# limanling/clip-event

Hardware: AMD Instinct MI355X
Metric: image-text pairs/sec/GPU, ViT-B/32 224px x 77-tok, global-batch contrastive (higher is better)
Workload: dtype bf16; 1 GPU; ViT-B/32 224px x 77-tok, bf16 operands, per-GPU batch 256, K=1, InfoNCE only, full train step (fwd+bwd+clip_grad_norm+Adam), random-init weights; global_batch=256, parallelism=dp1, captions=SOT + U[8,75] random ids + EOT, zero-padded to 77 (SURVEY 8(d) c2), text_rows=live tokens SOT..EOT only: 54.8% of B*77 rows (identical results, see DESIGN.md), fresh_captions_every_step=True, alignment=False, cu_hog=0, nt_pgrid=256, full=False

## Files before the change

clip_event_amd/csrc/gemm.hip:

```cpp
#include <stdlib.h>

#include <map>
#include <mutex>
#include <type_traits>

#include "common.hpp"
#include "nt_plan.hpp"
#include "tn_plan.hpp"
#include "../../include/clip_event_hip.h"

#ifndef CE_DIAG_TN3
#define CE_DIAG_TN3 0
#endif

namespace {

constexpr int NT_BM = 128, NT_BN = 128, NT_BK = 64;
constexpr int NT_STAGE_BYTES = (NT_BM + NT_BN) * NT_BK * 2;
constexpr int NT_LDS_BYTES = 2 * NT_STAGE_BYTES;

#include "gemm_common.hpp"

template <int EPI>
__global__ __launch_bounds__(256, 2) void gemm_nt_kernel(NTArgs p) {
// ... 970 lines not shown
            for (int it = 0; it < 2; ++it) {
                const int es = i * 2 + it;
                f32x4 v0 = *reinterpret_cast<const f32x4*>(ebuf + (it * 8 + e_r) * EROW + e_c * 4);
                f32x4 v1 = *reinterpret_cast<const f32x4*>(ebuf + (it * 8 + e_r) * EROW + e_c * 4 + 16);
                u32x4 a = {0u, 0u, 0u, 0u};
                if constexpr (PF_AUX) {
                    a = ap[es];
                }
                if constexpr (F8) {
                    const float sa = p.sa[min(m0 + e_row + es * 8, p.M - 1)];
                    v0 = v0 * sa * sb0;
                    v1 = v1 * sa * sb1;
                }
                v0 += bias0;
                v1 += bias1;
                if constexpr (EPI == CE_EPI_GELUGRAD_BF16) {
                    f32x4 r0 = {v0[0] * bf_lo(a[0]), v0[1] * bf_hi(a[0]), v0[2] * bf_lo(a[1]), v0[3] * bf_hi(a[1])};
                    f32x4 r1 = {v1[0] * bf_lo(a[2]), v1[1] * bf_hi(a[2]), v1[2] * bf_lo(a[3]), v1[3] * bf_hi(a[3])};
                    cs0 += r0;
                    cs1 += r1;
                    u32x4 o = {pack_bf2(r0[0], r0[1]), pack_bf2(r0[2], r0[3]), pack_bf2(r1[0], r1[1]), pack_bf2(r1[2], r1[3])};
                    epi_bstore16(eo, es, o);
                } else if constexpr (EPI == CE_EPI_BIAS_RESID_F16) {
                    v0 += f16x4_to_f32(u32x2{a[0], a[1]});
                    v1 += f16x4_to_f32(u32x2{a[2], a[3]});
                    const u32x2 h0 = f32_to_f16x4_sat(v0), h1 = f32_to_f16x4_sat(v1);
                    epi_bstore16(eo, es, u32x4{h0[0], h0[1], h1[0], h1[1]});
                } else {
                    nt_epilogue8b<EPI>(eo, eo2, er, es, v0, v1);
                }
            }
        }
        if constexpr (EPI == CE_EPI_GELUGRAD_BF16) {
            if (p.out2) {
                float* colsum = reinterpret_cast<float*>(p.out2);
#pragma unroll
                for (int e = 0; e < 4; ++e) {
#pragma unroll
                    for (int o = 8; o < 64; o <<= 1) {
                        cs0[e] += __shfl_xor(cs0[e], o, 64);
                        cs1[e] += __shfl_xor(cs1[e], o, 64);
                    }
                }
                const int e = lane >> 3;
                const float v = e == 0 ? cs0[0] : e == 1 ? cs0[1] : e == 2 ? cs0[2] : e == 3 ? cs0[3]
                              : e == 4 ? cs1[0] : e == 5 ? cs1[1] : e == 6 ? cs1[2] : cs1[3];
                if (gn + e < p.N) atomicAdd(colsum + gn + e, v);
            }
        }
    };
    for (; cur < list_end; ++t) {
        int tm, tn;
        persist_coords(p, cur, tm, tn);
        if constexpr (TS > 0) {
            if (tm < p.tall_panels) tile_body(std::integral_constant<int, TM>{}, tm, tn);
            else tile_body(std::integral_constant<int, TS>{}, tm, tn);
        } else {
            tile_body(std::integral_constant<int, TM>{}, tm, tn);
        }
        cur = dyn ? __builtin_amdgcn_readfirstlane(tq[(t + 1) & 1]) : cur + walk.step;
    }
}

constexpr int N3_BM = 160, N3_BN = 256, N3_BK = 32, N3_TM = 5;
constexpr int N3_A_BYTES = N3_BM * N3_BK * 2;
constexpr int N3_STAGE_BYTES = (N3_BM + N3_BN) * N3_BK * 2;
constexpr int N3_LDS_BYTES = 2 * N3_STAGE_BYTES;

template <int EPI>
__global__ __launch_bounds__(512, 4) void gemm_nt32_kernel(NTArgs p) {
    extern __shared__ __attribute__((aligned(16))) char smem[];
    const int tid = threadIdx.x;
    const int lane = tid & 63;
    const int wave = __builtin_amdgcn_readfirstlane(tid >> 6);
    const int wm = wave >> 2, wn = wave & 3;

    const int tile = xcd_remap(blockIdx.x, p.tiles_m * p.tiles_n);
    const int tm = tile / p.tiles_n, tn = tile - tm * p.tiles_n;
    const int m0 = tm * N3_BM, n0 = tn * N3_BN;
    const int rowsA = min(p.M - m0, N3_BM), rowsB = min(p.N - n0, N3_BN);
    const u32x4 rA = make_rsrc_words(p.A + (long)m0 * p.lda, (uint32_t)((long)rowsA * p.lda * 2));
    const u32x4 rB = make_rsrc_words(p.B + (long)n0 * p.ldb, (uint32_t)((long)rowsB * p.ldb * 2));

    const int s_row = lane >> 2;
    const int s_chunk = (lane & 3) ^ (((lane >> 5) & 1) << 1);
    const uint32_t vA0 = (uint32_t)((wave * 16 + s_row) * p.lda * 2 + s_chunk * 16);
    const uint32_t vA1 = (uint32_t)(((wave + 8) * 16 + s_row) * p.lda * 2 + s_chunk * 16);
    const uint32_t vB0 = (uint32_t)((wave * 16 + s_row) * p.ldb * 2 + s_chunk * 16);
    const uint32_t vB1 = (uint32_t)(((wave + 8) * 16 + s_row) * p.ldb * 2 + s_chunk * 16);
    const uint32_t lds0 = (uint32_t)(size_t)(lptr_t*)smem;
    auto stage = [&](int st, int kt) {
        const uint32_t base = lds0 + st * N3_STAGE_BYTES;
        const uint32_t kb = (uint32_t)(kt * N3_BK * 2);
        dma16_bounds(rA, base + wave * 1024, vA0 + kb);
        if (wave < 2) dma16_bounds(rA, base + (wave + 8) * 1024, vA1 + kb);
        dma16_bounds(rB, base + N3_A_BYTES + wave * 1024, vB0 + kb);
        dma16_bounds(rB, base + N3_A_BYTES + (wave + 8) * 1024, vB1 + kb);
    };

    f32x4 acc[N3_TM][4];
#pragma unroll
    for (int i = 0; i < N3_TM; ++i)
#pragma unroll
        for (int j = 0; j < 4; ++j) acc[i][j] = f32x4{0.f, 0.f, 0.f, 0.f};

    const int f_pos = (lane >> 4) ^ (((lane >> 3) & 1) << 1);
    const int fa_base = (wm * (N3_TM * 16) + (lane & 15)) * 64 + f_pos * 16;
    const int fb_base = N3_A_BYTES + (wn * 64 + (lane & 15)) * 64 + f_pos * 16;

    const int nk = p.K / N3_BK;
    stage(0, 0);
    asm volatile("s_waitcnt vmcnt(0)" ::: "memory");
    __syncthreads();
    for (int kt = 0; kt < nk; ++kt) {
        const int cur = kt & 1;
        if (kt + 1 < nk) stage(cur ^ 1, kt + 1);
        const char* st = smem + cur * N3_STAGE_BYTES;
        bf16x8 wf[4], af[N3_TM];
#pragma unroll
        for (int t = 0; t < 4; ++t) wf[t] = *reinterpret_cast<const bf16x8*>(st + fb_base + t * 1024);
#pragma unroll
        for (int t = 0; t < N3_TM; ++t) af[t] = *reinterpret_cast<const bf16x8*>(st + fa_base + t * 1024);
#pragma unroll
        for (int t = 0; t < N3_TM; ++t)
#pragma unroll
            for (int nt = 0; nt < 4; ++nt)
                acc[t][nt] = __builtin_amdgcn_mfma_f32_16x16x32_bf16(wf[nt], af[t], acc[t][nt], 0, 0, 0);
        asm volatile("s_waitcnt vmcnt(0)" ::: "memory");
        __syncthreads();
    }

    constexpr int EROW = 272;
    char* ebuf = smem + wave * (16 * EROW);
    const int e_r = lane >> 3, e_c = (lane & 7) * 8;
    const int gn = n0 + wn * 64 + e_c;
    f32x4 bias0 = {0.f, 0.f, 0.f, 0.f}, bias1 = {0.f, 0.f, 0.f, 0.f};
    f32x4 cs0 = {0.f, 0.f, 0.f, 0.f}, cs1 = {0.f, 0.f, 0.f, 0.f};
    if constexpr (epi_has_bias(EPI)) {
        if (gn < p.N) {
            bias0 = *reinterpret_cast<const f32x4*>(p.bias + gn);
            bias1 = *reinterpret_cast<const f32x4*>(p.bias + gn + 4);
        }
    }
#pragma unroll
    for (int t = 0; t < N3_TM; ++t) {
#pragma unroll
        for (int nt = 0; nt < 4; ++nt)
            *reinterpret_cast<f32x4*>(ebuf + (lane & 15) * EROW + (nt * 16 + 4 * (lane >> 4)) * 4) = acc[t][nt];
#pragma unroll
        for (int it = 0; it < 2; ++it) {
            const int m = m0 + wm * (N3_TM * 16) + t * 16 + it * 8 + e_r;
            f32x4 v0 = *reinterpret_cast<const f32x4*>(ebuf + (it * 8 + e_r) * EROW + e_c * 4);
            f32x4 v1 = *reinterpret_cast<const f32x4*>(ebuf + (it * 8 + e_r) * EROW + e_c * 4 + 16);
            if (m < p.M && gn < p.N) {
                v0 += bias0;
                v1 += bias1;
                nt_epilogue8<EPI>(p, m, gn, v0, v1, cs0, cs1);
            }
        }
    }
    if constexpr (EPI == CE_EPI_GELUGRAD_BF16) {
        if (p.out2) wg_colsum_flush(smem, reinterpret_cast<float*>(p.out2), n0, p.N, gn - n0, wm * 8 + e_r, cs0, cs1);
    }
}

constexpr int TN_BN = 128, TN_BK = 128, TN_BM = 64;
constexpr int TN_ROW = 320;
constexpr int TN_TILE_BYTES = TN_BM * TN_ROW;
constexpr int TN_STAGE_BYTES = 2 * TN_TILE_BYTES;
constexpr int TN_LDS_BYTES = 2 * TN_STAGE_BYTES;

struct TNArgs {
    const bf16_t* P; long ldp;
    const bf16_t* Q; long ldq;
    float* out; long ldo;
    int M, Nn, Kk;
    int tiles_n, tiles_k, splits, m_per_split;
};

__device__ __forceinline__ bf16x8 tr_frag(const char* tile, int byte_off) {
    typedef __attribute__((address_space(3))) s16x4 lds_s16x4;
    s16x4 lo = __builtin_amdgcn_ds_read_tr16_b64_v4i16((lds_s16x4*)(tile + byte_off));
    s16x4 hi = __builtin_amdgcn_ds_read_tr16_b64_v4i16((lds_s16x4*)(tile + byte_off + 4 * TN_ROW));
    typedef __attribute__((ext_vector_type(8))) short s16x8;
    s16x8 v = {lo[0], lo[1], lo[2], lo[3], hi[0], hi[1], hi[2], hi[3]};
    return __builtin_bit_cast(bf16x8, v);
}

__global__ __launch_bounds__(256, 2) void gemm_tn_kernel(TNArgs p) {
    extern __shared__ __attribute__((aligned(16))) char smem[];
    const int tid = threadIdx.x;
    const int lane = tid & 63;
    const int wave = __builtin_amdgcn_readfirstlane(tid >> 6);
    const int wn = wave >> 1, wk = wave & 1;

    int bid = blockIdx.x;
    const int split = bid % p.splits;
    bid /= p.splits;
    const int tk = bid % p.tiles_k, tn = bid / p.tiles_k;
    const int n0 = tn * TN_BN, k0 = tk * TN_BK;
    const int ms = split * p.m_per_split;
    const int me = min(p.M, ms + p.m_per_split);
    if (ms >= me) return;
    const int rows = me - ms;

    __amdgpu_buffer_rsrc_t rP = make_rsrc(p.P + (long)ms * p.ldp, (uint32_t)((long)rows * p.ldp * 2));
    __amdgpu_buffer_rsrc_t rQ = make_rsrc(p.Q + (long)ms * p.ldq, (uint32_t)((long)rows * p.ldq * 2));

    const int s_c = tid & 15, s_row = tid >> 4;
    const bool pvalid = (n0 + s_c * 8) < p.Nn, qvalid = (k0 + s_c * 8) < p.Kk;
    const uint32_t gP0 = (uint32_t)(s_row * p.ldp * 2 + (n0 + s_c * 8) * 2);
    const uint32_t gQ0 = (uint32_t)(s_row * p.ldq * 2 + (k0 + s_c * 8) * 2);
    const uint32_t gPstep = (uint32_t)(16 * p.ldp * 2), gQstep = (uint32_t)(16 * p.ldq * 2);
    const int lds_w = s_row * TN_ROW + s_c * 16;

    u32x4 rp[4], rq[4];
    auto issue_loads = [&](int mt) {
        const uint32_t mbP = (uint32_t)((long)mt * TN_BM * p.ldp * 2);
        const uint32_t mbQ = (uint32_t)((long)mt * TN_BM * p.ldq * 2);
#pragma unroll
        for (int i = 0; i < 4; ++i) {
            u32x4 z = {0u, 0u, 0u, 0u};
            rp[i] = pvalid ? __builtin_amdgcn_raw_buffer_load_b128(rP, gP0 + i * gPstep + mbP, 0, 0) : z;
            rq[i] = qvalid ? __builtin_amdgcn_raw_buffer_load_b128(rQ, gQ0 + i * gQstep + mbQ, 0, 0) : z;
        }
    };
    auto write_stage = [&](int stage) {
        char* sp = smem + stage * TN_STAGE_BYTES;
        char* sq = sp + TN_TILE_BYTES;
#pragma unroll
        for (int i = 0; i < 4; ++i) {
            *reinterpret_cast<u32x4*>(sp + lds_w + i * 16 * TN_ROW) = rp[i];
            *reinterpret_cast<u32x4*>(sq + lds_w + i * 16 * TN_ROW) = rq[i];
        }
    };

    f32x16 acc[2][2];
#pragma unroll
    for (int i = 0; i < 2; ++i)
#pragma unroll
        for (int j = 0; j < 2; ++j)
#pragma unroll
            for (int r = 0; r < 16; ++r) acc[i][j][r] = 0.f;

    const int g = lane >> 4, li = lane & 15;
    const int t_off = (8 * (g >> 1) + (li >> 2)) * TN_ROW + (16 * (g & 1) + 4 * (li & 3)) * 2;
    const int tp_base = t_off + (wn * 64) * 2;
    const int tq_base = TN_TILE_BYTES + t_off + (wk * 64) * 2;

    const int nmt = (rows + TN_BM - 1) / TN_BM;
    issue_loads(0);
    write_stage(0);
    __syncthreads();
    for (int mt = 0; mt < nmt; ++mt) {
        const int cur = mt & 1;
        if (mt + 1 < nmt) issue_loads(mt + 1);
        const char* st = smem + cur * TN_STAGE_BYTES;
#pragma unroll
        for (int s = 0; s < 4; ++s) {
            bf16x8 pf[2], qf[2];
#pragma unroll
            for (int t = 0; t < 2; ++t) {
                pf[t] = tr_frag(st, tp_base + s * 16 * TN_ROW + t * 64);
                qf[t] = tr_frag(st, tq_base + s * 16 * TN_ROW + t * 64);
            }
#pragma unroll
            for (int nt = 0; nt < 2; ++nt)
#pragma unroll
                for (int kt = 0; kt < 2; ++kt)
                    acc[nt][kt] = __builtin_amdgcn_mfma_f32_32x32x16_bf16(pf[nt], qf[kt], acc[nt][kt], 0, 0, 0);
        }
        if (mt + 1 < nmt) write_stage(cur ^ 1);
        __syncthreads();
    }

    const int ek = k0 + wk * 64 + (lane & 31);
    const int en = n0 + wn * 64 + 4 * (lane >> 5);
#pragma unroll
    for (int nt = 0; nt < 2; ++nt)
#pragma unroll
        for (int kt = 0; kt < 2; ++kt) {
            const int k = ek + kt * 32;
            if (k >= p.Kk) continue;
#pragma unroll
            for (int r = 0; r < 16; ++r) {
                const int n = en + nt * 32 + (r & 3) + 8 * (r >> 2);
                if (n < p.Nn) atomicAdd(p.out + (long)n * p.ldo + k, acc[nt][kt][r]);
            }
        }
}

constexpr int T2_TILE_BYTES = TN_BM * 256;
constexpr int T2_STAGE_BYTES = 2 * T2_TILE_BYTES;
constexpr int T2_LDS_BYTES = 2 * T2_STAGE_BYTES;

__device__ __forceinline__ bf16x8 tr_frag2(const char* p) {
    typedef __attribute__((address_space(3))) s16x4 lds_s16x4;
    s16x4 lo = __builtin_amdgcn_ds_read_tr16_b64_v4i16((lds_s16x4*)(p));
    s16x4 hi = __builtin_amdgcn_ds_read_tr16_b64_v4i16((lds_s16x4*)(p + 4 * 256));
    typedef __attribute__((ext_vector_type(8))) short s16x8;
    s16x8 v = {lo[0], lo[1], lo[2], lo[3], hi[0], hi[1], hi[2], hi[3]};
    return __builtin_bit_cast(bf16x8, v);
}

struct TNGroup {
    int count, splits, m_per_split, M, depth;
    int overwrite = 0;
    int tile_end[CE_TN_MAX_GROUP];
    TNArgs prob[CE_TN_MAX_GROUP];
};

__global__ __launch_bounds__(256, 2) void gemm_tn2_kernel(TNGroup grp) {
    extern __shared__ __attribute__((aligned(16))) char smem[];
    const int tid = threadIdx.x;
    const int lane = tid & 63;
    const int wave = __builtin_amdgcn_readfirstlane(tid >> 6);
    const int wn = wave >> 1, wk = wave & 1;

    const int m_tiles = (grp.M + TN_BM - 1) / TN_BM;
    const int mps = grp.m_per_split / TN_BM;
    const int s_r = lane >> 4;
    const int s_chunk = (lane & 15) ^ (s_r << 2);
    const int g = lane >> 4, li = lane & 15;
    const int t_row = 8 * (g >> 1) + (li >> 2);
    const int t_sw = (li >> 2) << 2;
    const int t_cb = 2 * (g & 1) + ((li & 3) >> 1);
    int offP[2], offQ[2];
#pragma unroll
    for (int t = 0; t < 2; ++t) {
        offP[t] = t_row * 256 + (((wn * 8 + t * 4 + t_cb) ^ t_sw) << 4) + (li & 1) * 8;
        offQ[t] = T2_TILE_BYTES + t_row * 256 + (((wk * 8 + t * 4 + t_cb) ^ t_sw) << 4) + (li & 1) * 8;
    }

    {
        const int lb = xcd_remap(blockIdx.x, gridDim.x);
        int tile = lb / grp.splits;
        const int mt0 = (lb - tile * grp.splits) * mps;
        const int mt1 = min(m_tiles, mt0 + mps);
        if (mt0 >= mt1) return;
        int pi = 0;
        while (pi + 1 < grp.count && tile >= grp.tile_end[pi]) ++pi;
        if (pi > 0) tile -= grp.tile_end[pi - 1];
        const TNArgs& p = grp.prob[pi];
        int tn, tk;
        {
            constexpr int BNB = 4, BKB = 4;
            const int br = tile / (BNB * p.tiles_k);
            const int r0 = br * BNB, rows_b = min(BNB, p.tiles_n - r0);
            const int t1 = tile - br * BNB * p.tiles_k;
            const int bc = t1 / (rows_b * BKB);
            const int c0 = bc * BKB, cols_b = min(BKB, p.tiles_k - c0);
            const int t2 = t1 - bc * rows_b * BKB;
            tn = r0 + t2 / cols_b;
            tk = c0 + t2 % cols_b;
        }
        const int n0 = tn * TN_BN, k0 = tk * TN_BK;
        const int ms = mt0 * TN_BM;
        const int rows = min(grp.M, mt1 * TN_BM) - ms;
        const long ldp = p.ldp, ldq = p.ldq;

        const u32x4 rP = make_rsrc_words(p.P + (long)ms * ldp, (uint32_t)((long)rows * ldp * 2));
        const u32x4 rQ = make_rsrc_words(p.Q + (long)ms * ldq, (uint32_t)((long)rows * ldq * 2));
        uint32_t vP[4], vQ[4];
#pragma unroll
        for (int j = 0; j < 4; ++j) {
            const int row = (wave * 4 + j) * 4 + s_r;
            vP[j] = (uint32_t)(row * ldp * 2 + (n0 + s_chunk * 8) * 2);
            vQ[j] = (uint32_t)(row * ldq * 2 + (k0 + s_chunk * 8) * 2);
        }
        const uint32_t lds0 = (uint32_t)(size_t)(lptr_t*)smem + wave * 4096;
        auto stage = [&](int st, int mt) {
            const uint32_t dp = lds0 + st * T2_STAGE_BYTES;
            const uint32_t dq = dp + T2_TILE_BYTES;
            const uint32_t mbP = (uint32_t)((long)mt * TN_BM * ldp * 2);
            const uint32_t mbQ = (uint32_t)((long)mt * TN_BM * ldq * 2);
#pragma unroll
            for (int j = 0; j < 4; ++j) {
                dma16_bounds(rP, dp + j * 1024, vP[j] + mbP);
                dma16_bounds(rQ, dq + j * 1024, vQ[j] + mbQ);
            }
        };

        f32x16 acc[2][2];
#pragma unroll
        for (int r = 0; r < 16; ++r) {
            acc[0][0][r] = 0.f; acc[0][1][r] = 0.f; acc[1][0][r] = 0.f; acc[1][1][r] = 0.f;
        }

        const int nmt = mt1 - mt0;
        stage(0, 0);
        asm volatile("s_waitcnt vmcnt(0)" ::: "memory");
        __syncthreads();
        for (int mt = 0; mt < nmt; ++mt) {
            const int cur = mt & 1;
            if (mt + 1 < nmt) stage(cur ^ 1, mt + 1);
            const char* st = smem + cur * T2_STAGE_BYTES;
#pragma unroll
            for (int s = 0; s < 4; ++s) {
                bf16x8 pf[2], qf[2];
#pragma unroll
                for (int t = 0; t < 2; ++t) {
                    pf[t] = tr_frag2(st + offP[t] + s * 16 * 256);
                    qf[t] = tr_frag2(st + offQ[t] + s * 16 * 256);
                }
#pragma unroll
                for (int nt = 0; nt < 2; ++nt)
#pragma unroll
                    for (int kt = 0; kt < 2; ++kt)
                        acc[nt][kt] = __builtin_amdgcn_mfma_f32_32x32x16_bf16(pf[nt], qf[kt], acc[nt][kt], 0, 0, 0);
            }
            asm volatile("s_waitcnt vmcnt(0)" ::: "memory");
            __syncthreads();
        }

        const int ek = k0 + wk * 64 + (lane & 31);
        const int en = n0 + wn * 64 + 4 * (lane >> 5);
        constexpr bool sole = false;
#pragma unroll
        for (int nt = 0; nt < 2; ++nt)
#pragma unroll
            for (int kt = 0; kt < 2; ++kt) {
                const int k = ek + kt * 32;
                if (k >= p.Kk) continue;
#pragma unroll
                for (int r = 0; r < 16; ++r) {
                    const int n = en + nt * 32 + (r & 3) + 8 * (r >> 2);
                    if (n < p.Nn) {
                        float* o = p.out + (long)n * p.ldo + k;
                        if (sole) *o += acc[nt][kt][r];
                        else atomicAdd(o, acc[nt][kt][r]);
                    }
                }
            }
    }
}

template <int T3_ROWS, int T3_STAGES>
__global__ __launch_bounds__(1024, 4) void gemm_tn3_kernel(TNGroup grp) {
    constexpr int T3_IMG_BYTES = T3_ROWS * 256;
    constexpr int T3_STAGE_BYTES = 4 * T3_IMG_BYTES;
    constexpr int KSTEPS = T3_ROWS / 16;
    constexpr int DPW = T3_ROWS / 16;
    extern __shared__ __attribute__((aligned(16))) char smem[];
    const int tid = threadIdx.x;
    const int lane = tid & 63;
    const int wave = __builtin_amdgcn_readfirstlane(tid >> 6);
    const int wn = wave >> 2, wk = wave & 3;

    const int m_tiles = (grp.M + TN_BM - 1) / TN_BM;
    const int mps = grp.m_per_split / TN_BM;
    const int s_r = lane >> 4;
    const int s_chunk = (lane & 15) ^ (s_r << 2);
    const int g = lane >> 4, li = lane & 15;
    const int t_row = 8 * (g >> 1) + (li >> 2);
    const int t_sw = (li >> 2) << 2;
    const int t_cb = 2 * (g & 1) + ((li & 3) >> 1);
    int offP[2], offQ[2];
#pragma unroll
    for (int t = 0; t < 2; ++t) {
        offP[t] = (wn >> 1) * T3_IMG_BYTES + t_row * 256 + ((((wn & 1) * 8 + t * 4 + t_cb) ^ t_sw) << 4) + (li & 1) * 8;
        offQ[t] = (2 + (wk >> 1)) * T3_IMG_BYTES + t_row * 256 + ((((wk & 1) * 8 + t * 4 + t_cb) ^ t_sw) << 4) + (li & 1) * 8;
    }

    const int lb = xcd_remap(blockIdx.x, gridDim.x);
    int tile = lb / grp.splits;
    const int mt0 = (lb - tile * grp.splits) * mps;
    const int mt1 = min(m_tiles, mt0 + mps);
    if (mt0 >= mt1) return;
    int pi = 0;
    while (pi + 1 < grp.count && tile >= grp.tile_end[pi]) ++pi;
    if (pi > 0) tile -= grp.tile_end[pi - 1];
    const TNArgs& p = grp.prob[pi];
    int tn, tk;
    {
        constexpr int BNB = 2, BKB = 2;
        const int br = tile / (BNB * p.tiles_k);
        const int r0 = br * BNB, rows_b = min(BNB, p.tiles_n - r0);
        const int t1 = tile - br * BNB * p.tiles_k;
        const int bc = t1 / (rows_b * BKB);
        const int c0 = bc * BKB, cols_b = min(BKB, p.tiles_k - c0);
        const int t2 = t1 - bc * rows_b * BKB;
        tn = r0 + t2 / cols_b;
        tk = c0 + t2 % cols_b;
    }
    const int n0 = tn * 256, k0 = tk * 256;
    const int ms = mt0 * TN_BM;
    const int rows = min(grp.M, mt1 * TN_BM) - ms;

    const int img = wave >> 2;
    const bool isP = img < 2;
    const long ld = isP ? p.ldp : p.ldq;
    const bf16_t* src = isP ? p.P : p.Q;
    const int col0 = (isP ? n0 : k0) + 128 * (img & 1);
    const u32x4 rsrc = make_rsrc_words(src + (long)ms * ld, (uint32_t)((long)rows * ld * 2));
    uint32_t vo[DPW];
#pragma unroll
    for (int j = 0; j < DPW; ++j) {
        const int row = ((wave & 3) * DPW + j) * 4 + s_r;
        vo[j] = (uint32_t)(row * ld * 2 + (col0 + s_chunk * 8) * 2);
    }
    const uint32_t lds0 = (uint32_t)(size_t)(lptr_t*)smem + img * T3_IMG_BYTES + (wave & 3) * DPW * 1024;
    auto stage = [&](int slot, int st) {
        const uint32_t d = lds0 + slot * T3_STAGE_BYTES;
        const uint32_t mb = (uint32_t)((long)st * T3_ROWS * ld * 2);
#pragma unroll
        for (int j = 0; j < DPW; ++j) dma16_bounds(rsrc, d + j * 1024, vo[j] + mb);
    };

    f32x16 acc[2][2];
#pragma unroll
    for (int r = 0; r < 16; ++r) {
        acc[0][0][r] = 0.f; acc[0][1][r] = 0.f; acc[1][0][r] = 0.f; acc[1][1][r] = 0.f;
    }

    const int nst = (rows + T3_ROWS - 1) / T3_ROWS;
    const int D = min(grp.depth, T3_STAGES - 1);
    stage(0, 0);
    if (nst > 1 && D > 1) stage(1, 1);
    if (nst > 2 && D > 2) stage(2, 2);
    int slot = 0;
    for (int i = 0; i < nst; ++i) {
        const int later = min(nst - 1 - i, D - 1);
        if (later == 2) asm volatile("s_waitcnt vmcnt(%0)" ::"n"(2 * DPW) : "memory");
        else if (later == 1) asm volatile("s_waitcnt vmcnt(%0)" ::"n"(DPW) : "memory");
        else asm volatile("s_waitcnt vmcnt(0)" ::: "memory");
        __builtin_amdgcn_s_barrier();
        if (i + D < nst) {
            int sl = slot + D;
            if (sl >= T3_STAGES) sl -= T3_STAGES;
            stage(sl, i + D);
        }
        const char* st = smem + slot * T3_STAGE_BYTES;
        slot = slot + 1 == T3_STAGES ? 0 : slot + 1;
#pragma unroll
        for (int s = 0; s < KSTEPS; ++s) {
            bf16x8 pf[2], qf[2];
#pragma unroll
            for (int t = 0; t < 2; ++t) {
                pf[t] = tr_frag2(st + offP[t] + s * 16 * 256);
                qf[t] = tr_frag2(st + offQ[t] + s * 16 * 256);
            }
#pragma unroll
            for (int nt = 0; nt < 2; ++nt)
#pragma unroll
                for (int kt = 0; kt < 2; ++kt)
                    acc[nt][kt] = __builtin_amdgcn_mfma_f32_32x32x16_bf16(pf[nt], qf[kt], acc[nt][kt], 0, 0, 0);
        }
    }

    const int ek = k0 + wk * 64 + (lane & 31);
    const int en = n0 + wn * 64 + 4 * (lane >> 5);
#pragma unroll
    for (int nt = 0; nt < 2; ++nt)
#pragma unroll
        for (int kt = 0; kt < 2; ++kt) {
            const int k = ek + kt * 32;
#pragma unroll
            for (int r = 0; r < 16; ++r) {
                const int n = en + nt * 32 + (r & 3) + 8 * (r >> 2);
                if (grp.overwrite) __builtin_nontemporal_store(acc[nt][kt][r], p.out + (long)n * p.ldo + k);
                else atomicAdd(p.out + (long)n * p.ldo + k, acc[nt][kt][r]);
            }
        }
}

template <int T3_ROWS, int T3_STAGES>
__global__ __launch_bounds__(768, 3) void gemm_tn3lw_kernel(TNGroup grp) {
    constexpr int T3_IMG_BYTES = T3_ROWS * 256;
    constexpr int T3_STAGE_BYTES = 4 * T3_IMG_BYTES;
    constexpr int KSTEPS = T3_ROWS / 16;
    constexpr int DPL = T3_ROWS / 4;
    extern __shared__ __attribute__((aligned(16))) char smem[];
    const int tid = threadIdx.x;
    const int lane = tid & 63;
    const int wave = __builtin_amdgcn_readfirstlane(tid >> 6);
    const int wn = (wave >> 2) & 1, wk = wave & 3;

    const int m_tiles = (grp.M + TN_BM - 1) / TN_BM;
    const int mps = grp.m_per_split / TN_BM;
    const int s_r = lane >> 4;
    const int s_chunk = (lane & 15) ^ (s_r << 2);
    const int g = lane >> 4, li = lane & 15;
    const int t_row = 8 * (g >> 1) + (li >> 2);
    const int t_sw = (li >> 2) << 2;
    const int t_cb = 2 * (g & 1) + ((li & 3) >> 1);
    int offP[4], offQ[2];
#pragma unroll
    for (int t = 0; t < 4; ++t)
        offP[t] = wn * T3_IMG_BYTES + t_row * 256 + (((t * 4 + t_cb) ^ t_sw) << 4) + (li & 1) * 8;
#pragma unroll
    for (int t = 0; t < 2; ++t)
        offQ[t] = (2 + (wk >> 1)) * T3_IMG_BYTES + t_row * 256 + ((((wk & 1) * 8 + t * 4 + t_cb) ^ t_sw) << 4) + (li & 1) * 8;

    const int lb = xcd_remap(blockIdx.x, gridDim.x);
    int tile = lb / grp.splits;
    const int mt0 = (lb - tile * grp.splits) * mps;
    const int mt1 = min(m_tiles, mt0 + mps);
    if (mt0 >= mt1) return;
    int pi = 0;
    while (pi + 1 < grp.count && tile >= grp.tile_end[pi]) ++pi;
    if (pi > 0) tile -= grp.tile_end[pi - 1];
    const TNArgs& p = grp.prob[pi];
    int tn, tk;
    {
        constexpr int BNB = 2, BKB = 2;
        const int br = tile / (BNB * p.tiles_k);
        const int r0 = br * BNB, rows_b = min(BNB, p.tiles_n - r0);
        const int t1 = tile - br * BNB * p.tiles_k;
        const int bc = t1 / (rows_b * BKB);
        const int c0 = bc * BKB, cols_b = min(BKB, p.tiles_k - c0);
        const int t2 = t1 - bc * rows_b * BKB;
        tn = r0 + t2 / cols_b;
        tk = c0 + t2 % cols_b;
    }
    const int n0 = tn * 256, k0 = tk * 256;
    const int ms = mt0 * TN_BM;
    const int rows = min(grp.M, mt1 * TN_BM) - ms;

    const int nst = (rows + T3_ROWS - 1) / T3_ROWS;
    const int D = min(grp.depth, T3_STAGES - 1);
    if (wave >= 8) {
        const int img = wave - 8;
        const bool isP = img < 2;
        const long ld = isP ? p.ldp : p.ldq;
        const bf16_t* src = isP ? p.P : p.Q;
        const int col0 = (isP ? n0 : k0) + 128 * (img & 1);
        const u32x4 rsrc = make_rsrc_words(src + (long)ms * ld, (uint32_t)((long)rows * ld * 2));
        const uint32_t vo0 = (uint32_t)(s_r * ld * 2 + (col0 + s_chunk * 8) * 2);
        const uint32_t vstep = (uint32_t)(4 * ld * 2);
        const uint32_t lds0 = (uint32_t)(size_t)(lptr_t*)smem + img * T3_IMG_BYTES;
        auto stage = [&](int slot, int st) {
            const uint32_t d = lds0 + slot * T3_STAGE_BYTES;
            const uint32_t mb = (uint32_t)((long)st * T3_ROWS * ld * 2);
#pragma unroll
            for (int j = 0; j < DPL; ++j) {
#if CE_DIAG_TN3 == 2
                if (p.ldo < 0)
#endif
                dma16_bounds(rsrc, d + j * 1024, vo0 + j * vstep + mb);
            }
        };
        stage(0, 0);
        if (nst > 1 && D > 1) stage(1, 1);
        if (nst > 2 && D > 2) stage(2, 2);
        int slot = 0;
        for (int i = 0; i < nst; ++i) {
            const int later = min(nst - 1 - i, D - 1);
            if (later == 2) asm volatile("s_waitcnt vmcnt(%0)" ::"n"(2 * DPL) : "memory");
            else if (later == 1) asm volatile("s_waitcnt vmcnt(%0)" ::"n"(DPL) : "memory");
            else asm volatile("s_waitcnt vmcnt(0)" ::: "memory");
            __builtin_amdgcn_s_barrier();
            if (i + D < nst) {
                int sl = slot + D;
                if (sl >= T3_STAGES) sl -= T3_STAGES;
                stage(sl, i + D);
            }
            slot = slot + 1 == T3_STAGES ? 0 : slot + 1;
        }
        return;
    }

    f32x16 acc[4][2];
#pragma unroll
    for (int nt = 0; nt < 4; ++nt)
#pragma unroll
        for (int r = 0; r < 16; ++r) {
            acc[nt][0][r] = 0.f; acc[nt][1][r] = 0.f;
        }
    int slot = 0;
    for (int i = 0; i < nst; ++i) {
        __builtin_amdgcn_s_barrier();
        const char* st = smem + slot * T3_STAGE_BYTES;
        slot = slot + 1 == T3_STAGES ? 0 : slot + 1;
#pragma unroll
        for (int s = 0; s < KSTEPS; ++s) {
            bf16x8 qf[2];
#pragma unroll
            for (int t = 0; t < 2; ++t) qf[t] = tr_frag2(st + offQ[t] + s * 16 * 256);
#pragma unroll
            for (int nt = 0; nt < 4; ++nt) {
                const bf16x8 pf = tr_frag2(st + offP[nt] + s * 16 * 256);
#pragma unroll
                for (int kt = 0; kt < 2; ++kt)
                    acc[nt][kt] = __builtin_amdgcn_mfma_f32_32x32x16_bf16(pf, qf[kt], acc[nt][kt], 0, 0, 0);
            }
        }
    }

    const int ek = k0 + wk * 64 + (lane & 31);
    const int en = n0 + wn * 128 + 4 * (lane >> 5);
#pragma unroll
    for (int nt = 0; nt < 4; ++nt)
#pragma unroll
        for (int kt = 0; kt < 2; ++kt) {
            const int k = ek + kt * 32;
#pragma unroll
            for (int r = 0; r < 16; ++r) {
                const int n = en + nt * 32 + (r & 3) + 8 * (r >> 2);
#if CE_DIAG_TN3 == 1
                if (acc[nt][kt][r] == 12345.678f)
#endif
                if (grp.overwrite) __builtin_nontemporal_store(acc[nt][kt][r], p.out + (long)n * p.ldo + k);
                else atomicAdd(p.out + (long)n * p.ldo + k, acc[nt][kt][r]);
            }
        }
}

__global__ void probe_mfma16_kernel(const bf16x8* a, const bf16x8* b, f32x4* out) {
    f32x4 c = {0.f, 0.f, 0.f, 0.f};
    c = __builtin_amdgcn_mfma_f32_16x16x32_bf16(a[threadIdx.x], b[threadIdx.x], c, 0, 0, 0);
    out[threadIdx.x] = c;
}
__global__ void probe_mfma32_kernel(const bf16x8* a, const bf16x8* b, f32x16* out) {
    f32x16 c;
#pragma unroll
    for (int r = 0; r < 16; ++r) c[r] = 0.f;
    c = __builtin_amdgcn_mfma_f32_32x32x16_bf16(a[threadIdx.x], b[threadIdx.x], c, 0, 0, 0);
    out[threadIdx.x] = c;
}
__global__ void probe_tr16_kernel(const uint16_t* image, int n_elems, const int* byte_off, s16x4* out) {
    extern __shared__ __attribute__((aligned(16))) char smem[];
    uint16_t* l = reinterpret_cast<uint16_t*>(smem);
    for (int i = threadIdx.x; i < n_elems; i += 64) l[i] = image[i];
    __syncthreads();
    typedef __attribute__((address_space(3))) s16x4 lds_s16x4;
    out[threadIdx.x] = __builtin_amdgcn_ds_read_tr16_b64_v4i16((lds_s16x4*)(smem + byte_off[threadIdx.x]));
}

static_assert(NT_PLAN_LDS[NT_NT128] == NT_LDS_BYTES && NT_PLAN_LDS[NT_NT256x2] == N2H_LDS_BYTES && NT_PLAN_LDS[NT_NT256x4] == N2_LDS_BYTES &&
              NT_PLAN_LDS[NT_NT32] == N3_LDS_BYTES && NT_PLAN_LDS[NT_NT160_RING] == N4_LDS_BYTES && NT_PLAN_LDS[NT_LW] == N4_LDS_BYTES &&
              NT_PLAN_LDS[NT_PERSIST] == N4P_LDS_BYTES && NT_PLAN_LDS[NT_SKINNY] == SK_LDS_BYTES &&
              NT_PLAN_BLOCK[NT_LW] == 64 * (8 + N4_LOADERS), "nt_plan.hpp is out of step with the kernels");

int env_int(const char* name, int otherwise) {
    const char* e = getenv(name);
    return e ? atoi(e) : otherwise;
}
NTKnobs knobs_from_env() {
    NTKnobs k;
    k.cus = env_int("CE_GEMM_CUS", 256);
    k.dynamic = env_int("CE_NT_DYNAMIC", 0);
    k.env_chunk = env_int("CE_NT_CHUNK", 0);
    k.env_pgrid = env_int("CE_NT_PGRID", 0);
    k.env_mixed = env_int("CE_NT_MIXED", 1);
    return k;
}
NTKnobs g_knobs = knobs_from_env();
NTPlan g_last_plan;

struct TileQueueRing { unsigned int* dev = nullptr; int next = 0; };
constexpr int TQ_RING = 1024;
std::mutex g_tq_mu;
std::map<hipStream_t, TileQueueRing> g_tq;
unsigned int* next_tile_queue(hipStream_t s) {
    std::lock_guard<std::mutex> lk(g_tq_mu);
    TileQueueRing& r = g_tq[s];
    if (!r.dev) {
        if (hipMalloc(&r.dev, TQ_RING * sizeof(unsigned int)) != hipSuccess) return nullptr;
        r.next = TQ_RING;
    }
    if (r.next >= TQ_RING) {
        if (hipMemsetAsync(r.dev, 0, TQ_RING * sizeof(unsigned int), s) != hipSuccess) return nullptr;
        r.next = 0;
    }
    return r.dev + r.next++;
}

template <auto Kernel, class Args>
void launch_kernel(int workgroups, int block, int lds_bytes, const Args& a, hipStream_t stream) {
    static std::once_flag attr;
    std::call_once(attr, [&] {
        hipFuncSetAttribute(reinterpret_cast<const void*>(Kernel), hipFuncAttributeMaxDynamicSharedMemorySize, lds_bytes);
    });
    hipLaunchKernelGGL(Kernel, dim3(workgroups), dim3(block), lds_bytes, stream, a);
}

template <int EPI, int F8>
bool dispatch(const NTPlan& p, const NTArgs& a, hipStream_t s) {
#define CE_NT_CASE_IF(COND, KERNEL, TM, TS, ...) \
    case key(KERNEL, TM, TS): if constexpr (COND) { launch_kernel<__VA_ARGS__>(p.workgroups, p.block, p.lds_bytes, a, s); return true; } break
#define CE_NT_CASE(KERNEL, TM, ...) CE_NT_CASE_IF(true, KERNEL, TM, 0, __VA_ARGS__)
    constexpr auto key = [](int kernel, int tm, int ts) { return 128 * kernel + 8 * tm + ts; };
    constexpr bool two = nt_two_heights(EPI);
    if constexpr (F8) {
        switch (key(p.kernel, p.tm, p.ts)) {
            CE_NT_CASE(NT_LW, 5, gemm_nt160lw_kernel<EPI, 5, 1>);
            CE_NT_CASE(NT_LW, 4, gemm_nt160lw_kernel<EPI, 4, 1>);
            CE_NT_CASE(NT_LW, 3, gemm_nt160lw_kernel<EPI, 3, 1>);
            CE_NT_CASE(NT_PERSIST, 4, gemm_nt160p_kernel<EPI, 4, 1>);
            CE_NT_CASE_IF(two, NT_PERSIST, 4, 1, gemm_nt160p_kernel<EPI, 4, 1, 1>);
            CE_NT_CASE_IF(two, NT_PERSIST, 4, 2, gemm_nt160p_kernel<EPI, 4, 1, 2>);
            CE_NT_CASE_IF(two, NT_PERSIST, 4, 3, gemm_nt160p_kernel<EPI, 4, 1, 3>);
            CE_NT_CASE(NT_PERSIST, 3, gemm_nt160p_kernel<EPI, 3, 1>);
        }
    } else {
        switch (key(p.kernel, p.tm, p.ts)) {
            CE_NT_CASE(NT_NT128, 4, gemm_nt_kernel<EPI>);
            CE_NT_CASE(NT_NT256x2, 5, gemm_nt256_kernel<EPI, 5, 2>);
            CE_NT_CASE(NT_NT32, 5, gemm_nt32_kernel<EPI>);
            CE_NT_CASE(NT_NT160_RING, 5, gemm_nt160_kernel<EPI>);
            CE_NT_CASE(NT_LW, 5, gemm_nt160lw_kernel<EPI, 5>);
            CE_NT_CASE(NT_LW, 4, gemm_nt160lw_kernel<EPI, 4>);
            CE_NT_CASE(NT_LW, 3, gemm_nt160lw_kernel<EPI, 3>);
            CE_NT_CASE(NT_PERSIST, 5, gemm_nt160p_kernel<EPI, 5>);
            CE_NT_CASE(NT_PERSIST, 4, gemm_nt160p_kernel<EPI, 4>);
            CE_NT_CASE(NT_PERSIST, 3, gemm_nt160p_kernel<EPI, 3>);
            CE_NT_CASE_IF(two, NT_PERSIST, 5, 1, gemm_nt160p_kernel<EPI, 5, 0, 1>);
            CE_NT_CASE_IF(two, NT_PERSIST, 5, 2, gemm_nt160p_kernel<EPI, 5, 0, 2>);
            CE_NT_CASE_IF(two, NT_PERSIST, 5, 3, gemm_nt160p_kernel<EPI, 5, 0, 3>);
            CE_NT_CASE_IF(two, NT_PERSIST, 5, 4, gemm_nt160p_kernel<EPI, 5, 0, 4>);
            CE_NT_CASE(NT_NT256x2, 3, gemm_nt256_kernel<EPI, 3, 2>);
            CE_NT_CASE(NT_NT256x2, 4, gemm_nt256_kernel<EPI, 4, 2>);
            CE_NT_CASE(NT_NT256x4, 3, gemm_nt256_kernel<EPI, 3, 4>);
            CE_NT_CASE(NT_NT256x4, 4, gemm_nt256_kernel<EPI, 4, 4>);
            CE_NT_CASE(NT_NT256x4, 5, gemm_nt256_kernel<EPI, 5, 4>);
            CE_NT_CASE(NT_NT256x4, 6, gemm_nt256_kernel<EPI, 6, 4>);
            CE_NT_CASE(NT_NT256x4, 7, gemm_nt256_kernel<EPI, 7, 4>);
            CE_NT_CASE(NT_NT256x4, 8, gemm_nt256_kernel<EPI, 8, 4>);
            CE_NT_CASE(NT_SKINNY, 2, gemm_nt_skinny_kernel<EPI>);
        }
    }
#undef CE_NT_CASE
#undef CE_NT_CASE_IF
    return false;
}

template <int EPI, int F8>
int launch_nt(NTArgs a, hipStream_t stream) {
    const NTPlan p = nt_plan(NTShape{a.M, a.N, a.K, a.lda, a.ldb, a.ldo, a.ldo2, a.ldaux, a.ldr}, EPI, F8, g_knobs);
    if (!p.taken) return 1;
    CE_CHECK_ARG(!(p.needs_colsum_pass && a.out2) || (a.N % 8 == 0 && a.ldo % 8 == 0),
                 "ce_gemm_nt: GELUGRAD column sums on the 128x128 kernel need N and ldo multiples of 8 (N=%d ldo=%ld)", a.N, a.ldo);
    g_last_plan = p;
    const double operand_bytes = (F8 ? 1.0 : 2.0) * ((double)a.M * a.K + (double)a.N * a.K);
    CeProfScope prof(nt_prof_class(EPI) + p.family, 2.0 * a.M * a.N * a.K, operand_bytes + epi_traffic_bytes(EPI) * a.M * a.N, stream);
    a.tiles_m = p.tiles_m; a.tiles_n = p.tiles_n; a.tall_panels = p.tall_panels; a.tile_chunk = p.tile_chunk;
    a.tile_queue = p.wants_tile_queue ? next_tile_queue(stream) : nullptr;
    CE_CHECK_ARG((dispatch<EPI, F8>(p, a, stream)), "ce_gemm_nt: no kernel %d with tile heights %d, %d (epilogue %d, fp8 %d)", (int)p.kernel,
                 p.tm, p.ts, EPI, F8);
    CE_LAUNCH_CHECK();
    if (p.needs_colsum_pass && a.out2) return ce_colsum_bf16(a.out, a.ldo, reinterpret_cast<float*>(a.out2), a.M, a.N, stream);
    return 0;
}

}

extern "C" int ce__gemm_nt_fp8_lw(const void* A8, long lda, const float* sa, const void* B8, long ldb, const float* sb, int M, int N,
                                  int K, int epilogue, const float* bias, const void* resid, long ldr, void* out, long ldo,
                                  void* out2, long ldo2, const void* aux, long ldaux, void* stream) {
    NTArgs a;
    a.A = (const bf16_t*)A8; a.lda = lda; a.B = (const bf16_t*)B8; a.ldb = ldb;
    a.M = M; a.N = N; a.K = K; a.bias = bias; a.resid = (const float*)resid; a.ldr = ldr;
    a.out = out; a.ldo = ldo; a.out2 = (bf16_t*)out2; a.ldo2 = ldo2; a.aux = (const bf16_t*)aux; a.ldaux = ldaux;
    a.sa = sa; a.sb = sb;
    hipStream_t s = (hipStream_t)stream;
    switch (epilogue) {
        case CE_EPI_BF16: return launch_nt<CE_EPI_BF16, 1>(a, s);
        case CE_EPI_BIAS_BF16: return launch_nt<CE_EPI_BIAS_BF16, 1>(a, s);
        case CE_EPI_BIAS_RESID_F32: return launch_nt<CE_EPI_BIAS_RESID_F32, 1>(a, s);
        case CE_EPI_BIAS_RESID_F16: return launch_nt<CE_EPI_BIAS_RESID_F16, 1>(a, s);
        case CE_EPI_BIAS_GELU: return launch_nt<CE_EPI_BIAS_GELU, 1>(a, s);
        case CE_EPI_BIAS_QGELU_BF16: return launch_nt<CE_EPI_BIAS_QGELU_BF16, 1>(a, s);
        case CE_EPI_GELUGRAD_BF16: return launch_nt<CE_EPI_GELUGRAD_BF16, 1>(a, s);
        default: return 1;
    }
}

extern "C" int ce_gemm_set_dynamic_tiles(int on) {
    g_knobs.dynamic = on < 0 ? knobs_from_env().dynamic : (on != 0);
    return 0;
}

extern "C" int ce_gemm_set_cu_budget(int cus) {
    CE_CHECK_ARG(cus == 0 || (cus >= 32 && cus <= 256), "ce_gemm_set_cu_budget: 32..256 CUs, or 0 for the default (CE_GEMM_CUS / 256)");
    g_knobs.cus = cus ? cus : knobs_from_env().cus;
    return 0;
}

extern "C" int ce_gemm_nt_plan(int M, int N, int K, int epilogue, int fp8, long lda, long ldb, long ldo, long ldo2, long ldaux,
                               long ldr, ce_nt_plan* out) {
    CE_CHECK_ARG(out && M > 0 && N > 0 && K > 0, "ce_gemm_nt_plan: empty problem M=%d N=%d K=%d, or no result struct", M, N, K);
    CE_CHECK_ARG(epilogue >= CE_EPI_BF16 && epilogue <= CE_EPI_BIAS_QGELU_BF16, "ce_gemm_nt_plan: unknown epilogue %d", epilogue);
    const NTPlan p = nt_plan(NTShape{M, N, K, lda, ldb, ldo, ldo2, ldaux, ldr}, epilogue, fp8 != 0, g_knobs);
    *out = ce_nt_plan{p.kernel, p.tm, p.ts, p.tall_panels, p.tiles_m, p.tiles_n, p.tile_chunk, p.workgroups, p.block, p.lds_bytes,
                      p.wants_tile_queue, p.taken};
    return 0;
}

extern "C" int ce_gemm_nt_last_plan(int* tall_panels, int* short_tm) {
    if (tall_panels) *tall_panels = g_last_plan.tall_panels;
    if (short_tm) *short_tm = g_last_plan.ts;
    return 0;
}

extern "C" void ce_gemm_nt_tune(int variant) {
    if (variant >= 1000 && variant < 2000) g_knobs.force_chunk = variant - 1001;
    else g_knobs.force_tile = variant < 0 ? 0 : variant;
}

extern "C" int ce_gemm_nt(const void* A, long lda, const void* B, long ldb, int M, int N, int K, int epilogue,
                          const float* bias, const void* resid, long ldr, void* out, long ldo, void* out2,
                          long ldo2, const void* aux, long ldaux, void* stream) {
    CE_CHECK_ARG(M > 0 && N > 0 && K > 0, "ce_gemm_nt: empty problem M=%d N=%d K=%d", M, N, K);
    CE_CHECK_ARG(K % 8 == 0 && N % 4 == 0, "ce_gemm_nt: need K%%8==0 and N%%4==0 (K=%d N=%d)", K, N);
    CE_CHECK_ARG(lda % 8 == 0 && ldb % 8 == 0 && ldo % 4 == 0, "ce_gemm_nt: lda/ldb must be multiples of 8, ldo of 4");
    CE_CHECK_ARG(lda >= K && ldb >= K && ldo >= N, "ce_gemm_nt: leading dimension smaller than the row");
    CE_CHECK_ARG(128L * lda * 2 < (1L << 32) && 128L * ldb * 2 < (1L << 32), "ce_gemm_nt: row panel exceeds 4 GiB");
    NTArgs a;
    a.A = (const bf16_t*)A; a.lda = lda; a.B = (const bf16_t*)B; a.ldb = ldb;
    a.M = M; a.N = N; a.K = K; a.bias = bias; a.resid = (const float*)resid; a.ldr = ldr;
    a.out = out; a.ldo = ldo; a.out2 = (bf16_t*)out2; a.ldo2 = ldo2; a.aux = (const bf16_t*)aux; a.ldaux = ldaux;
    hipStream_t s = (hipStream_t)stream;
    switch (epilogue) {
        case CE_EPI_BF16: return launch_nt<CE_EPI_BF16, 0>(a, s);
        case CE_EPI_F32: return launch_nt<CE_EPI_F32, 0>(a, s);
        case CE_EPI_BIAS_BF16:
            CE_CHECK_ARG(bias, "ce_gemm_nt: bias epilogue without bias");
            return launch_nt<CE_EPI_BIAS_BF16, 0>(a, s);
        case CE_EPI_BIAS_F32:
            CE_CHECK_ARG(bias, "ce_gemm_nt: bias epilogue without bias");
            return launch_nt<CE_EPI_BIAS_F32, 0>(a, s);
        case CE_EPI_BIAS_RESID_F32:
            CE_CHECK_ARG(bias && resid && ldr >= N && ldr % 4 == 0, "ce_gemm_nt: residual epilogue needs bias+resid");
            return launch_nt<CE_EPI_BIAS_RESID_F32, 0>(a, s);
        case CE_EPI_BIAS_RESID_F16:
            CE_CHECK_ARG(bias && resid && ldr >= N && ldr % 8 == 0 && ldo % 8 == 0, "ce_gemm_nt: fp16 residual epilogue needs bias+resid, ldr/ldo multiples of 8");
            return launch_nt<CE_EPI_BIAS_RESID_F16, 0>(a, s);
        case CE_EPI_BIAS_GELU:
            CE_CHECK_ARG(bias && out2 && ldo2 >= N && ldo2 % 4 == 0, "ce_gemm_nt: gelu epilogue needs bias+out2");
            return launch_nt<CE_EPI_BIAS_GELU, 0>(a, s);
        case CE_EPI_BIAS_QGELU_BF16:
            CE_CHECK_ARG(bias, "ce_gemm_nt: QuickGELU epilogue without bias");
            return launch_nt<CE_EPI_BIAS_QGELU_BF16, 0>(a, s);
        case CE_EPI_GELUGRAD_BF16:
            CE_CHECK_ARG(aux && ldaux >= N && ldaux % 4 == 0, "ce_gemm_nt: gelu-grad epilogue needs aux");
            return launch_nt<CE_EPI_GELUGRAD_BF16, 0>(a, s);
        default: CE_CHECK_ARG(false, "ce_gemm_nt: unknown epilogue %d", epilogue);
    }
    return 0;
}

extern "C" int ce_gemm_tn(const void* P, long ldp, const void* Q, long ldq, int M, int Nn, int Kk, float* out,
                          long ldo, int splits, void* stream) {
    return ce_gemm_tn_bias(P, ldp, Q, ldq, M, Nn, Kk, out, ldo, nullptr, splits, stream);
}

extern "C" int ce_gemm_tn_bias(const void* P, long ldp, const void* Q, long ldq, int M, int Nn, int Kk, float* out,
                               long ldo, float* bias_grad, int splits, void* stream) {
    const void* Ps[1] = {P};
    const void* Qs[1] = {Q};
    float* outs[1] = {out};
    int rc = ce_gemm_tn_grouped(1, Ps, &ldp, Qs, &ldq, M, &Nn, &Kk, outs, &ldo, splits, stream);
    if (rc != 0) return rc;
    if (bias_grad) return ce_colsum_bf16(P, ldp, bias_grad, M, Nn, stream);
    return 0;
}

extern "C" int ce_gemm_tn_grouped(int count, const void* const* P, const long* ldp, const void* const* Q,
                                  const long* ldq, int M, const int* Nn, const int* Kk, float* const* out,
                                  const long* ldo, int splits, void* stream) {
    return ce_gemm_tn_grouped_ex(count, P, ldp, Q, ldq, M, Nn, Kk, out, ldo, splits, 0, stream);
}

static_assert(TN_PLAN_BM == TN_BM && TN_PLAN_LDS_V1 == TN_LDS_BYTES && TN_PLAN_LDS_128 == T2_LDS_BYTES &&
              tn_plan_lds_256(48, 3) == 3 * 48 * 1024 && tn_plan_lds_256(32, 4) == 4 * 32 * 1024 && TN_PLAN_BLOCK[TN_V1] == 256 &&
              TN_PLAN_BLOCK[TN_V2] == 256 && TN_PLAN_BLOCK[TN_V3] == 1024 && TN_PLAN_BLOCK[TN_V3LW] == 768,
              "tn_plan.hpp is out of step with the kernels");

extern "C" int ce_gemm_tn_grouped_ex(int count, const void* const* P, const long* ldp, const void* const* Q,
                                     const long* ldq, int M, const int* Nn, const int* Kk, float* const* out,
                                     const long* ldo, int splits, int overwrite, void* stream) {
    CE_CHECK_ARG(count >= 1 && count <= CE_TN_MAX_GROUP && M > 0, "ce_gemm_tn_grouped: 1..%d problems, M > 0", CE_TN_MAX_GROUP);
    hipStream_t s = (hipStream_t)stream;
    TNGroup g;
    g.count = count;
    g.M = M;
    double flops = 0.0, bytes = 0.0;
    long ldmax = 0;
    for (int i = 0; i < count; ++i) {
        CE_CHECK_ARG(Nn[i] > 0 && Kk[i] > 0, "ce_gemm_tn: empty problem");
        CE_CHECK_ARG(Nn[i] % 8 == 0 && Kk[i] % 8 == 0 && ldp[i] % 8 == 0 && ldq[i] % 8 == 0,
                     "ce_gemm_tn: Nn,Kk,ldp,ldq must be multiples of 8");
        CE_CHECK_ARG(ldp[i] >= Nn[i] && ldq[i] >= Kk[i] && ldo[i] >= Kk[i], "ce_gemm_tn: leading dimension smaller than the row");
        TNArgs& a = g.prob[i];
        a.P = (const bf16_t*)P[i]; a.ldp = ldp[i]; a.Q = (const bf16_t*)Q[i]; a.ldq = ldq[i];
        a.out = out[i]; a.ldo = ldo[i]; a.M = M; a.Nn = Nn[i]; a.Kk = Kk[i];
        flops += 2.0 * M * Nn[i] * Kk[i];
        bytes += 2.0 * ((double)M * Nn[i] + (double)M * Kk[i]) + 8.0 * Nn[i] * Kk[i];
        if (ldp[i] > ldmax) ldmax = ldp[i];
        if (ldq[i] > ldmax) ldmax = ldq[i];
    }
    CE_CHECK_ARG((long)M * ldmax * 2 < (1L << 32), "ce_gemm_tn: operand exceeds 4 GiB");

// ... 70 lines not shown
```

Baseline: 21290 pairs/s (whole job).

## Software-pipeline LDS transposed reads against MFMAs in TN3 GEMM main loop

Rewrites the TN3 kernel's inner loop as a software pipeline. P and Q fragments are read from LDS a couple of pairs ahead into a small register ring, and the last MFMA pair of each stage is deferred so it overlaps the next stage's first reads. It also switches to precomputed 32-bit LDS addresses advanced by a stride per stage, and uses sched_barriers plus an explicit lgkmcnt wait to force the interleaving. The aim is to hide ds_read_tr latency behind MFMAs. The cost is more register pressure and rigid scheduling that could hurt occupancy.

```diff
diff --git a/clip_event_amd/csrc/gemm.hip b/clip_event_amd/csrc/gemm.hip
--- a/clip_event_amd/csrc/gemm.hip
+++ b/clip_event_amd/csrc/gemm.hip
@@ -1296,6 +1296,14 @@
     s16x8 v = {lo[0], lo[1], lo[2], lo[3], hi[0], hi[1], hi[2], hi[3]};
     return __builtin_bit_cast(bf16x8, v);
 }
+__device__ __forceinline__ bf16x8 tr_frag2_lds(uint32_t a) {
+    typedef __attribute__((address_space(3))) s16x4 lds_s16x4;
+    s16x4 lo = __builtin_amdgcn_ds_read_tr16_b64_v4i16((lds_s16x4*)(size_t)a);
+    s16x4 hi = __builtin_amdgcn_ds_read_tr16_b64_v4i16((lds_s16x4*)(size_t)(a + 4 * 256));
+    typedef __attribute__((ext_vector_type(8))) short s16x8;
+    s16x8 v = {lo[0], lo[1], lo[2], lo[3], hi[0], hi[1], hi[2], hi[3]};
+    return __builtin_bit_cast(bf16x8, v);
+}
 
 struct TNGroup {
     int count, splits, m_per_split, M, depth;
@@ -1661,28 +1669,57 @@
         for (int r = 0; r < 16; ++r) {
             acc[nt][0][r] = 0.f; acc[nt][1][r] = 0.f;
         }
+    constexpr int NPAIR = 4 * KSTEPS, RING = 2;
+    constexpr int QC = (KSTEPS - 1) & 1;
+    typedef __attribute__((ext_vector_type(8))) short s16x8;
+    const bf16x8 zero8 = __builtin_bit_cast(bf16x8, s16x8{0, 0, 0, 0, 0, 0, 0, 0});
+    bf16x8 pb[RING], qf[2][2];
+    pb[(NPAIR - 1) % RING] = zero8; qf[QC][0] = zero8; qf[QC][1] = zero8;
+    const uint32_t ring0 = (uint32_t)(size_t)(lptr_t*)smem;
+    uint32_t aP[4], aQ[2];
+#pragma unroll
+    for (int t = 0; t < 4; ++t) aP[t] = ring0 + (uint32_t)offP[t];
+#pragma unroll
+    for (int t = 0; t < 2; ++t) aQ[t] = ring0 + (uint32_t)offQ[t];
+    auto read_p = [&](int j) { return tr_frag2_lds(aP[j % 4] + (j / 4) * 16 * 256); };
+    auto pair = [&](int j, const bf16x8& q0, const bf16x8& q1) {
+        acc[j % 4][0] = __builtin_amdgcn_mfma_f32_32x32x16_bf16(pb[j % RING], q0, acc[j % 4][0], 0, 0, 0);
+        acc[j % 4][1] = __builtin_amdgcn_mfma_f32_32x32x16_bf16(pb[j % RING], q1, acc[j % 4][1], 0, 0, 0);
+    };
     int slot = 0;
     for (int i = 0; i < nst; ++i) {
+        asm volatile("s_waitcnt lgkmcnt(0)" ::: "memory");
         __builtin_amdgcn_s_barrier();
-        const char* st = smem + slot * T3_STAGE_BYTES;
+        const bf16x8 qc0 = qf[QC][0], qc1 = qf[QC][1];
+        qf[0][0] = tr_frag2_lds(aQ[0]); qf[0][1] = tr_frag2_lds(aQ[1]);
+        pb[0] = read_p(0);
+        __builtin_amdgcn_sched_barrier(0);
+        pair(NPAIR - 1, qc0, qc1);
+        pb[1] = read_p(1);
+        __builtin_amdgcn_sched_barrier(0);
+#pragma unroll
+        for (int j = 0; j < NPAIR - 1; ++j) {
+            const int s = j / 4;
+            if (j % 4 == 0 && s + 1 < KSTEPS) {
+                qf[(s + 1) & 1][0] = tr_frag2_lds(aQ[0] + (s + 1) * 16 * 256);
+                qf[(s + 1) & 1][1] = tr_frag2_lds(aQ[1] + (s + 1) * 16 * 256);
+            }
+            pair(j, qf[s & 1][0], qf[s & 1][1]);
+            if (j + RING < NPAIR) pb[j % RING] = read_p(j + RING);
+            __builtin_amdgcn_sched_barrier(0);
+        }
+        const uint32_t step = slot + 1 == T3_STAGES ? (uint32_t)(-(T3_STAGES - 1) * T3_STAGE_BYTES) : (uint32_t)T3_STAGE_BYTES;
         slot = slot + 1 == T3_STAGES ? 0 : slot + 1;
 #pragma unroll
-        for (int s = 0; s < KSTEPS; ++s) {
-            bf16x8 qf[2];
-#pragma unroll
-            for (int t = 0; t < 2; ++t) qf[t] = tr_frag2(st + offQ[t] + s * 16 * 256);
-#pragma unroll
-            for (int nt = 0; nt < 4; ++nt) {
-                const bf16x8 pf = tr_frag2(st + offP[nt] + s * 16 * 256);
-#pragma unroll
-                for (int kt = 0; kt < 2; ++kt)
-                    acc[nt][kt] = __builtin_amdgcn_mfma_f32_32x32x16_bf16(pf, qf[kt], acc[nt][kt], 0, 0, 0);
-            }
-        }
-    }
-
-    const int ek = k0 + wk * 64 + (lane & 31);
-    const int en = n0 + wn * 128 + 4 * (lane >> 5);
+        for (int t = 0; t < 4; ++t) aP[t] += step;
+#pragma unroll
+        for (int t = 0; t < 2; ++t) aQ[t] += step;
+    }
+    pair(NPAIR - 1, qf[QC][0], qf[QC][1]);
+
+    const int el = __builtin_amdgcn_mbcnt_hi(~0u, __builtin_amdgcn_mbcnt_lo(~0u, 0u));
+    const int ek = k0 + wk * 64 + (el & 31);
+    const int en = n0 + wn * 128 + 4 * (el >> 5);
 #pragma unroll
     for (int nt = 0; nt < 4; ++nt)
 #pragma unroll
```

After: 21230 pairs/s (whole job). About the same (-0.3%).
